# vsu/foo-dsp-bfir

Hardware: AMD Instinct MI355X
Metric: Msamples/s (output channel-samples), 8ch 131072-tap FIR @4096-sample partitions (higher is better)
Workload: dtype f32; 1 GPU; cfg3_8ch_131072tap_L4096_fp32; channels=8, taps=131072, partition=4096, fft_size=8192, partitions=32, blocks_per_launch=4096, engines_rank0=1, channels_rank0=8, streams_total=1, io=interleaved frames resident in HBM (generated there), parallelism=one independent stream per rank, no collective

## Files before the change

### foo-dsp-bfir_amd/csrc/engine.hip

```cpp
#include <hip/hip_runtime.h>

#include <algorithm>
#include <climits>
#include <cmath>
#include <cstdarg>
#include <cstdio>
#include <cstdlib>
#include <cstring>
#include <cstdint>
#include <thread>
#include <type_traits>
#include <vector>

#include "../../include/bfir_hip.h"
#include "kernels.h"

using namespace bfir;

static bfir_log_fn g_log = nullptr;

extern "C" void bfir_set_log_callback(bfir_log_fn fn) { g_log = fn; }

void bfir_logf(const char *fmt, ...)
{
// ... 54 lines not shown
    int Co = 0, GCo = 0;
    bool mimo = false, mimo_mac = false;
    int in_bytes = 0, out_bytes = 0, in_fmt = 0, out_fmt = 0;
    double in_scale = 1.0, out_scale = 1.0, of_max = 1.0;
    FftPlan plan;
    bool big = false;
    BigPlan bplan;
    int chunk = 0, ring = 0;
    int want_chunk = 0;
    void *H = nullptr, *X = nullptr, *Y = nullptr, *tout = nullptr;
    void *tin[2] = {nullptr, nullptr};
    void *Yb[2] = {nullptr, nullptr};
    void *saved[2] = {nullptr, nullptr};
    BlockRef hist[2];
    int *d_nblk = nullptr;
    DevOverflow *d_of = nullptr;
    int *d_bad = nullptr;
    std::vector<int> nblk;
    std::vector<char> eng_init;
    unsigned long long blockcounter = 0;
    unsigned long long chunk_seq = 0;
    int curbuf = 0;
    hipStream_t stream = nullptr, s_front = nullptr, s_mac = nullptr, s_in = nullptr, s_out = nullptr;
    hipEvent_t ev_entry = nullptr, ev_fwd[2] = {nullptr, nullptr}, ev_mac[2] = {nullptr, nullptr};
    hipEvent_t ev_inv[2] = {nullptr, nullptr};
    bool pipe3 = true;
    bool ilv = false;
    bool pair = false;
    bool pair_tp = false;
    bool pair_cap = false;
    bool direct = false;
    FftPlan plan2;
    void *H2 = nullptr;
    int *d_nblk2 = nullptr;
    std::vector<int> nblk2;
    int fade_len = 0, fade_pos = 0;
    float fade_f = 0.f; double fade_d = 0.0;
    bool fade_fused = false;
    bool pair_new = false;
    bool fade_patch = false;
    int *d_patch = nullptr; size_t patch_ints = 0;
    bool patch_fused = false;
    void *bank = nullptr;
    std::vector<int> bank_nb;
    int *d_gather = nullptr; size_t gather_ints = 0;
    void *Yf[2] = {nullptr, nullptr};
    int yf_blocks = 0;
    void *ft[2] = {nullptr, nullptr};
    int ft_blocks = 0;
    float *tails[2][2] = {{nullptr, nullptr}, {nullptr, nullptr}};
    const float *hist_raw[2] = {nullptr, nullptr};
    int8_t *d_dither_tab = nullptr; int dither_size = 0;
    DevDitherState *d_dither_state = nullptr;
    bool inline_launch = false;
    bool async_pending = false;
    int *h_bad = nullptr;
    int *bad_host_cur = nullptr;
    bool serial = false;
    void *pin_in[2] = {nullptr, nullptr}, *pin_out[2] = {nullptr, nullptr};
    void *dev_in[2] = {nullptr, nullptr}, *dev_out[2] = {nullptr, nullptr};
    hipEvent_t ev_h2d[2] = {nullptr, nullptr}, ev_comp[2] = {nullptr, nullptr}, ev_d2h[2] = {nullptr, nullptr};
    size_t stage_bytes_in = 0, stage_bytes_out = 0;
    bool nup = false, nup_tail = false;
    bool levels = false;
    bool mlevels = false;
    bool back_fused = false;
    int n_tail = 0;
    bfir_engine *tail[BFIR_MAX_LEVELS - 1] = {nullptr, nullptr, nullptr};
    int lv_r[BFIR_MAX_LEVELS - 1] = {0, 0, 0}, lv_D[BFIR_MAX_LEVELS - 1] = {0, 0, 0};
    bool lv_active[BFIR_MAX_LEVELS - 1] = {false, false, false};
    int nup_mask = 0;
    void *pbuf = nullptr;
    long long pbuf_upto = 0;
    hipEvent_t ev_nup = nullptr;
    void *zring = nullptr; int zblocks = 0;
    long long z_from = 0, z_next = 0;
    int ring_extra = 0;
    void *zring2 = nullptr;
    int lf_mode = 0; long long lf_j1 = -1;
    bool lf_stop = false;
    bool mfade_duo = true;
    int inv_quad = -1;
    int fwd_wide = -1;
    bool profiling = false;
    struct Span { int k; hipEvent_t a, b; };
    std::vector<Span> spans;
    std::vector<hipEvent_t> ev_pool;
    double prof_ms[BFIR_K_COUNT] = {0, 0, 0, 0, 0};
    long prof_n[BFIR_K_COUNT] = {0, 0, 0, 0, 0};
    struct DelaySide {
        bool on = false;
        int max_delay = 0, steps = 0, h = 0;
        double beta = 0.0;
        long H = 0;
        void *hist[2] = {nullptr, nullptr}; int cur = 0;
        void *scratch = nullptr; size_t scratch_bytes = 0;
        void *d_tab = nullptr;
        std::vector<int> delay, sub;
    };
    DelaySide dly[2];
    hipEvent_t ev_dly = nullptr;
    hipEvent_t ev_dly_done = nullptr; hipStream_t dly_stream = nullptr;
};

static size_t cbuf_bytes(const bfir_engine *e) { return (size_t)e->N * (size_t)e->s; }

static bfir_engine *level(const bfir_engine *e, int k) { return k == 0 ? const_cast<bfir_engine *>(e) : e->tail[k - 1]; }

static void delay_free(bfir_engine *e, int side)
{
    bfir_engine::DelaySide &d = e->dly[side];
    void *bufs[] = {d.hist[0], d.hist[1], d.scratch, d.d_tab};
    for (void *b : bufs) if (b) (void)hipFree(b);
    d = bfir_engine::DelaySide();
}

static int materialise_history(bfir_engine *e)
{
    HIP_TRY(hipDeviceSynchronize());
    const size_t Ls = (size_t)e->L * e->s;
    for (int i = 0; i < 2; i++) {
        if (e->hist[i].ptr != e->saved[i])
            HIP_TRY(hipMemcpy2D(e->saved[i], Ls, e->hist[i].ptr, (size_t)e->hist[i].ch_stride * e->s, Ls, e->GC,
                                hipMemcpyDeviceToDevice));
        e->hist[i].ptr = e->saved[i];
        e->hist[i].ch_stride = e->L;
    }
    HIP_TRY(hipDeviceSynchronize());
    return BFIR_OK;
}

static void free_staging(bfir_engine *e)
{
    for (int i = 0; i < 2; i++) {
        if (e->pin_in[i]) (void)hipHostFree(e->pin_in[i]);
        if (e->pin_out[i]) (void)hipHostFree(e->pin_out[i]);
        if (e->dev_in[i]) (void)hipFree(e->dev_in[i]);
        if (e->dev_out[i]) (void)hipFree(e->dev_out[i]);
        e->pin_in[i] = e->pin_out[i] = e->dev_in[i] = e->dev_out[i] = nullptr;
    }
    e->stage_bytes_in = e->stage_bytes_out = 0;
}

static void free_work(bfir_engine *e)
{
    void **bufs[] = {&e->X, &e->Yb[0], &e->Yb[1], &e->tin[0], &e->tin[1], &e->tout};
    for (void **b : bufs) { if (*b) (void)hipFree(*b); *b = nullptr; }
    free_staging(e);
    e->chunk = e->ring = 0;
    if (e->h_bad) { (void)hipHostFree(e->h_bad); e->h_bad = nullptr; }
}

static int alloc_work(bfir_engine *e, int chunk)
{
    const size_t cb = cbuf_bytes(e);
    const int ring = 2 * chunk + e->B + e->ring_extra;
    if (e->X) { int rc = materialise_history(e); if (rc != BFIR_OK) return rc; }
    void *X = nullptr, *Y0 = nullptr, *Y1 = nullptr, *tin0 = nullptr, *tin1 = nullptr, *tout = nullptr;
    HIP_TRY(hipMalloc(&X, (size_t)e->GC * ring * cb));
    HIP_TRY(hipMalloc(&Y0, (size_t)e->GCo * chunk * cb));
    HIP_TRY(hipMalloc(&Y1, (size_t)e->GCo * chunk * cb));
    if (e->nup && !e->back_fused) HIP_TRY(hipMalloc(&tout, (size_t)e->GCo * chunk * e->L * e->s));
    if (!e->pair && !e->direct) {
        HIP_TRY(hipMalloc(&tin0, (size_t)e->GC * chunk * e->L * e->s));
        HIP_TRY(hipMalloc(&tin1, (size_t)e->GC * chunk * e->L * e->s));
        HIP_TRY(hipMalloc(&tout, (size_t)e->GCo * chunk * e->L * e->s));
    }
    HIP_TRY(hipMemset(X, 0, (size_t)e->GC * ring * cb));
    if (e->X) {
        const int keep = (int)std::min<unsigned long long>(e->blockcounter, (unsigned long long)(e->B - 1 + e->ring_extra));
        for (int d = 1; d <= keep; d++) {
            const unsigned long long j = e->blockcounter - d;
            const size_t so = (size_t)(j % e->ring) * cb, dn = (size_t)(j % ring) * cb;
            HIP_TRY(hipMemcpy2D((char *)X + dn, (size_t)ring * cb, (char *)e->X + so, (size_t)e->ring * cb, cb,
                                e->GC, hipMemcpyDeviceToDevice));
        }
    }
    HIP_TRY(hipDeviceSynchronize());
    free_work(e);
    e->X = X; e->Yb[0] = Y0; e->Yb[1] = Y1; e->tin[0] = tin0; e->tin[1] = tin1; e->tout = tout;
    e->chunk = chunk; e->ring = ring;
    return BFIR_OK;
}

static void choose_path(bfir_engine *e)
{
    e->ilv = e->s == 4 && e->N >= 512;
    const char *pv = getenv("BFIR_PAIR");
    const char *tv = getenv("BFIR_PAIR_TIME");
    const bool tp_ok = !(tv && atoi(tv) == 0);
    e->pair_tp = (e->C % 2) == 1 && tp_ok;
    e->pair = e->ilv && e->in_fmt == 8 && e->out_fmt == 8 && ((e->C % 2) == 0 || e->pair_tp) &&
              pair_supported(e->L) && !(pv && atoi(pv) == 0);
    e->pair_tp = e->pair_tp && e->pair;
    if (e->matrix) {
        const bool split = e->nup || e->nup_tail;
        e->pair = e->pair && e->C % 2 == 0 && (split || e->Co % 2 == 0);
        e->pair_tp = false;
        e->pair_cap = e->pair;
    }
    const char *dv = getenv("BFIR_DIRECT");
    const bool stereo = e->in_bytes == 4 && e->out_bytes == 4 && (e->C % 2) == 0 && !e->ilv &&
                        direct_stereo_supported(e->L, e->s);
    const bool wide = (e->in_bytes == 8 && e->out_bytes == 8) || e->C == 1 || stereo || run64_supported(e->L, e->s);
    e->direct = !e->pair && fmt_is_native(e->in_fmt) && fmt_is_native(e->out_fmt) && !(pv && atoi(pv) == 0) &&
                (dv ? atoi(dv) != 0 : wide);
    if (e->matrix) e->direct = !e->pair;
    if (e->big) e->pair = e->pair_tp = e->direct = false;
    if (e->nup || e->nup_tail) {
        e->pair = e->pair && !e->pair_tp;
        e->pair_tp = false;
        e->direct = !e->pair;
        e->back_fused = e->nup && (e->matrix ? e->s == 4 && e->ilv && e->out_fmt == BFIR_SAMPLE_FORMAT_FLOAT_LE && pair_supported(e->L)
                                             : e->pair);
    }
    {
        const char *fp = getenv("BFIR_F64_PAIRS"), *ms = getenv("BFIR_MAC_SYS");
        const bool other_mac = (ms && atoi(ms) == 0) || getenv("BFIR_MAC_BATCHED");
        if (e->s == 8 && e->direct && pairs64_supported(e->L, e->s) && e->B <= BFIR_MAC_SYS_MAX_B && !other_mac &&
            !(fp && atoi(fp) == 0))
            e->ilv = true;
    }
    if (const char *mv = getenv("BFIR_MFADE_DUO")) e->mfade_duo = atoi(mv) != 0;
    if (const char *pf = getenv("BFIR_PATCH_FUSED")) e->patch_fused = atoi(pf) != 0;
    if (e->mimo) {
        const char *mm = getenv("BFIR_MIMO_MAC");
        e->mimo_mac = e->C > BFIR_MAT_MAX || e->Co > BFIR_MAT_MAX || (mm && atoi(mm) != 0);
    }
    if (const char *qv = getenv("BFIR_INV_QUAD")) e->inv_quad = atoi(qv) != 0;
    if (const char *wv = getenv("BFIR_FWD_WIDE")) e->fwd_wide = atoi(wv) != 0;
    if (const char *pm = getenv("BFIR_PIPE")) { e->pipe3 = atoi(pm) >= 3; e->serial = atoi(pm) == 1; }
    else if (e->s == 8) { e->pipe3 = false; e->serial = true; }
}

static void log_creation(const bfir_engine *e)
{
    char shape[64];
    if (e->big) {
        bfir_logf("bfir engine: big, %d x %d channels, partition %d = %d x %d, %d blocks, realsize %d on device %d. layout=%s",
                  e->n_eng, e->C, e->L, 1 << e->bplan.log2m1, 1 << e->bplan.log2m2, e->B, e->s, e->device, e->ilv ? "pairs" : "grouped");
        return;
    }
    if (e->matrix) snprintf(shape, sizeof(shape), "%s %d -> %d", e->mimo ? "mimo" : "matrix", e->C, e->Co);
    else snprintf(shape, sizeof(shape), "%d x %d channels", e->n_eng, e->C);
    bfir_logf("bfir engine: %s, partition %d, %d blocks, realsize %d on device %d. path=%s layout=%s run=%s",
              shape, e->L, e->B, e->s, e->device,
              e->pair_tp ? "time-pair" : e->pair ? "pair" : e->direct ? "direct" : "staging", e->ilv ? "pairs" : "grouped",
              e->s == 8 && e->direct && run64_supported(e->L, e->s) ? "on" : "off");
}

static bfir_engine *engine_create(int n_engines, int filter_length, int filter_blocks, int realsize, int channels,
                                  int channels_out, bool matrix, int in_format, int out_format, int sampling_rate,
                                  int apply_dither, int device, int *err, int nup_level = 0, int ring_extra = 0, bool big = false,
                                  int max_channels = BFIR_MAXCHANNELS)
{
    const bool mimo = matrix && max_channels > BFIR_MAXCHANNELS;
    int dummy;
    if (!err) err = &dummy;
    *err = BFIR_OK;
    if (channels < 1 || channels > max_channels || channels_out < 1 || channels_out > max_channels) {
        bfir_logf("Number of channels (%d) exceeds limit (%d).", std::max(channels, channels_out), max_channels);
        *err = BFIR_ERR_ARG; return nullptr;
    }
    if (realsize != 4 && realsize != 8) { bfir_logf("Invalid real size %d.", realsize); *err = BFIR_ERR_ARG; return nullptr; }
    if (filter_length < 1 || (filter_length & (filter_length - 1))) {
        bfir_logf("Invalid length %d.", filter_length); *err = BFIR_ERR_ARG; return nullptr;
    }
    if (filter_blocks < 1 || n_engines < 1) { *err = BFIR_ERR_ARG; return nullptr; }
    if (!fmt_bytes(in_format) || !fmt_bytes(out_format)) { *err = BFIR_ERR_UNSUPPORTED; return nullptr; }
    int ndev = bfir_device_count();
    if (ndev <= 0) { *err = BFIR_ERR_NO_DEVICE; return nullptr; }
    if (device < 0 || device >= ndev) { *err = BFIR_ERR_ARG; return nullptr; }
    if (hipSetDevice(device) != hipSuccess) { *err = BFIR_ERR_HIP; return nullptr; }

    bfir_engine *e = new bfir_engine();
    e->device = device;
    e->L = filter_length; e->N = 2 * filter_length; e->B = filter_blocks; e->s = realsize;
    e->C = channels; e->n_eng = n_engines; e->GC = n_engines * channels;
    e->matrix = matrix; e->Co = channels_out; e->GCo = n_engines * channels_out;
    e->mimo = mimo;
    e->in_bytes = fmt_bytes(in_format); e->out_bytes = fmt_bytes(out_format);
    e->in_fmt = in_format; e->out_fmt = out_format;
    e->in_scale = fmt_info(in_format).isfloat ? 1.0 : 1.0 / fmt_full_scale(in_format);
    e->out_scale = fmt_info(out_format).isfloat ? 1.0 : fmt_full_scale(out_format);
    e->of_max = fmt_info(out_format).isfloat ? 1.0 : fmt_full_scale(out_format) - 1.0;
    e->nup = nup_level == 1; e->nup_tail = nup_level == 2;
    e->ring_extra = ring_extra;
    e->big = big;
    choose_path(e);
    e->nblk.assign(matrix ? (size_t)e->Co * e->C : (size_t)e->GC, 0);
    e->eng_init.assign(n_engines, 0);
    int rc = big ? big_plan_create(&e->bplan, filter_length, realsize) : fft_plan_create(&e->plan, filter_length, realsize);
    if (rc != 0) { *err = (rc == -1) ? BFIR_ERR_UNSUPPORTED : BFIR_ERR_HIP; delete e; return nullptr; }
    auto fail = [&](int code) { *err = code; bfir_engine_destroy(e); return (bfir_engine *)nullptr; };
    if (e->pair || e->direct) {
        if ((e->pair || e->back_fused) && fft_plan_create(&e->plan2, 2 * filter_length, 4) != 0) return fail(BFIR_ERR_HIP);
        const size_t tb = (size_t)e->n_eng * e->L * e->C * e->in_bytes;
        for (int st = 0; st < 2; st++)
            for (int i = 0; i < 2; i++) {
                if (hipMalloc((void **)&e->tails[st][i], tb) != hipSuccess) return fail(BFIR_ERR_HIP);
                (void)hipMemset(e->tails[st][i], 0, tb);
            }
        e->hist_raw[0] = e->tails[1][0]; e->hist_raw[1] = e->tails[1][1];
    }
    hipStream_t *streams[] = {&e->stream, &e->s_front, &e->s_mac, &e->s_in, &e->s_out};
    for (hipStream_t *st : streams)
        if (hipStreamCreateWithFlags(st, hipStreamNonBlocking) != hipSuccess) return fail(BFIR_ERR_HIP);
    hipEvent_t *events[] = {&e->ev_entry, &e->ev_fwd[0], &e->ev_fwd[1], &e->ev_mac[0], &e->ev_mac[1],
                            &e->ev_inv[0], &e->ev_inv[1],
                            &e->ev_h2d[0], &e->ev_h2d[1], &e->ev_comp[0], &e->ev_comp[1], &e->ev_d2h[0], &e->ev_d2h[1]};
    for (hipEvent_t *ev : events)
        if (hipEventCreateWithFlags(ev, hipEventDisableTiming) != hipSuccess) return fail(BFIR_ERR_HIP);
    const size_t cb = cbuf_bytes(e), Ls = (size_t)e->L * e->s;
// ... 1370 lines not shown
    d.h2 = e->H2;
    d.row = e->d_patch; d.ent = e->d_patch + e->Co + 1;
    d.y2 = Y2; d.y2_ch_stride = y2_ch_stride;
    return d;
}

static int patch_chunk_ok(const bfir_engine *e, int tc)
{
    const long ys = (long)e->chunk * e->N;
    if (!patch_supported(patch_args(e, 0, nullptr, nullptr, 0, tc)) ||
        (chunk_takes_wpatch(e) && !wpatch_supported(wpatch_args(e, 0, nullptr, ys, nullptr, 0, tc)))) {
        bfir_logf("bfir engine: %d fading blocks per launch are past the pair-list kernel's grid.", tc);
        return BFIR_ERR_UNSUPPORTED;
    }
    return BFIR_OK;
}

static int queue_mac_patch(bfir_engine *e, int base_slot, void *Y, long y_ch_stride, void *Y2, long y2_ch_stride, int tc,
                           hipStream_t s, bool spans)
{
    const bool prof = e->profiling;
    if (!spans) e->profiling = false;
    int rc;
    if (chunk_takes_wpatch(e)) {
        ProfScope ps(e, BFIR_K_MAC, s);
        rc = launch_wpatch(wpatch_args(e, base_slot, Y, y_ch_stride, Y2, y2_ch_stride, tc), s) != 0 ? BFIR_ERR_UNSUPPORTED : BFIR_OK;
    } else {
        {
            ProfScope ps(e, BFIR_K_MAC, s);
            rc = queue_mac(e, base_slot, Y, y_ch_stride, tc, false, s);
        }
        if (rc == BFIR_OK) {
            ProfScope ps(e, BFIR_K_MAC, s);
            PatchArgs a = patch_args(e, base_slot, Y, Y2, y2_ch_stride, tc);
            a.y_ch_stride = y_ch_stride;
            rc = launch_patch(a, s) != 0 ? BFIR_ERR_UNSUPPORTED : BFIR_OK;
        }
    }
    e->profiling = prof;
    return rc;
}

static int chunk_aligned(const bfir_engine *e, Path p, const Chunk &c)
{
    const uintptr_t out_mask = (e->pair_tp || (e->matrix && (e->Co & 1))) ? 3 : 7;
    if (p == Path::Pair &&
        ((((uintptr_t)c.d_in | (uintptr_t)c.in_stride) & (e->pair_tp ? 3 : 7)) || (((uintptr_t)c.d_out | (uintptr_t)c.out_stride) & out_mask))) {
        bfir_logf("bfir engine: frame buffers of the float fast path must be 8-byte aligned (4 with an odd channel count).");
        return BFIR_ERR_ARG;
    }
    if (p == Path::Direct && (((uintptr_t)c.d_in | (uintptr_t)c.in_stride) % e->in_bytes ||
                              ((uintptr_t)c.d_out | (uintptr_t)c.out_stride) % e->out_bytes)) {
        bfir_logf("bfir engine: frame buffers must be aligned to their sample size.");
        return BFIR_ERR_ARG;
    }
    return BFIR_OK;
}

static void queue_stage_in(bfir_engine *e, const Chunk &c, hipStream_t sf)
{
    ProfScope ps(e, BFIR_K_STAGE_IN, sf);
    StageInArgs a;
    a.raw = c.d_in; a.eng_stride_bytes = c.in_stride; a.frame_off = c.frame_off;
    a.n_eng = e->n_eng; a.C = e->C; a.raw_bytes = e->in_bytes; a.spacing = e->C; a.fmt = e->in_fmt;
    a.n_frames = (long)c.tc * e->L;
    a.dst = e->tin[c.par]; a.dst_ch_stride = (long)e->chunk * e->L; a.dst_off = 0;
    a.realsize = e->s;
    launch_stage_in(a, sf);
}

static void queue_fwd(bfir_engine *e, Path p, const Chunk &c, hipStream_t sf)
{
    ProfScope ps(e, BFIR_K_FWD, sf);
    if (p == Path::Pair) {
        FwdPairArgs a;
        a.raw = (const float *)c.d_in; a.eng_stride = c.in_stride / 4; a.frame_off = c.frame_off;
        a.C = e->C; a.n_eng = e->n_eng; a.n_t = c.tc;
        a.prev = e->hist_raw[e->curbuf];
        a.save_last = e->tails[c.par][c.idx_last]; a.save_prev = e->tails[c.par][1 ^ c.idx_last];
        a.carry = e->hist_raw[1 ^ c.idx_last];
        a.hist_eng_stride = (long)e->L * e->C;
        a.dst = (float *)e->X; a.dst_ch_stride = (long)e->ring * e->N; a.ring = e->ring; a.base_slot = c.base_slot;
        a.scale = (float)e->in_scale;
        a.tp = e->pair_tp; a.wide = e->fwd_wide;
        launch_fwd_pair(e->plan2, a, sf);
    } else {
        FwdArgs a;
        a.dst = e->X; a.dst_ch_stride = (long)e->ring * e->N; a.ring = e->ring; a.base_slot = c.base_slot;
        a.n_t = c.tc; a.n_ch = e->GC;
        a.load_scale = 1.0; a.out_scale = e->in_scale; a.zero_first_half = 0; a.interleaved = e->ilv;
        if (p == Path::Direct) {
            a.src = nullptr; a.src_ch_stride = 0; a.prev = nullptr; a.prev_ch_stride = 0;
            a.raw_bytes = e->in_bytes; a.raw = c.d_in; a.raw_eng_stride = c.in_stride / e->in_bytes; a.frame_off = c.frame_off; a.C = e->C;
            a.prev_raw = e->hist_raw[e->curbuf];
            a.save_last = e->tails[c.par][c.idx_last]; a.save_prev = e->tails[c.par][1 ^ c.idx_last];
            a.carry = e->hist_raw[1 ^ c.idx_last];
            a.hist_eng_stride = (long)e->L * e->C;
        } else {
            a.src = e->tin[c.par]; a.src_ch_stride = (long)e->chunk * e->L;
            a.prev = e->hist[e->curbuf].ptr; a.prev_ch_stride = e->hist[e->curbuf].ch_stride;
        }
        queue_transform_fwd(e, a, sf);
    }
    if (p != Path::Staging) { e->hist_raw[0] = e->tails[c.par][0]; e->hist_raw[1] = e->tails[c.par][1]; }
}

static InvStats inv_stats(const bfir_engine *e, const Chunk &c)
{
    return InvStats{(float)e->of_max, e->d_of, e->GCo, e->d_bad, c.block_base, e->bad_host_cur};
}

static int chunk_rings(const bfir_engine *e, LevelRing (&ring)[BFIR_LEVEL_RINGS], const void **z_new = nullptr)
{
    int nr = 0;
    for (int i = 0; i < e->n_tail; i++) {
        if (!(e->nup_mask >> i & 1)) continue;
        const bfir_engine *t = e->tail[i];
        if (z_new) z_new[nr] = t->lf_mode ? t->zring2 : t->zring;
        LevelRing &g = ring[nr++];
        g.z = t->zring; g.zlen = g.z_ch_stride = (long)t->zblocks * t->L;
        g.m0 = ((long long)e->blockcounter - e->lv_D[i]) * e->L; g.m_min = t->z_from * (long long)t->L;
        g.m0r = (long)(((g.m0 % g.zlen) + g.zlen) % g.zlen);
    }
    if (!nr) ring[0] = LevelRing{nullptr, 0, 0, 0, 0, 0};
    for (int k = std::max(nr, 1); k < BFIR_LEVEL_RINGS; k++) { ring[k] = ring[0]; if (z_new) z_new[k] = z_new[0]; }
    return nr;
}

static void queue_inv_lone(bfir_engine *e, const Chunk &c, const LevelRing (&ring)[BFIR_LEVEL_RINGS], int nr, hipStream_t st)
{
    LoneInvArgs a;
    a.ch = e->Co & ~1;
    a.y = (const float *)c.Y + (long)a.ch * e->chunk * e->N;
    for (int k = 0; k < BFIR_LEVEL_RINGS; k++) a.ring[k] = ring[k];
    a.n_rings = nr;
    a.raw = (float *)c.d_out; a.frame_off = c.frame_off;
    a.frame_stride = e->Co; a.n_t = c.tc;
    a.scale = (float)e->out_scale; a.st = inv_stats(e, c);
    launch_inv_lone(e->plan2, a, st);
}

static void queue_inv(bfir_engine *e, Path p, const Chunk &c, hipStream_t st)
{
    ProfScope ps(e, BFIR_K_INV, st);
    if (p == Path::Pair) {
        InvPairArgs a;
        a.y = (const float *)c.Y; a.y_ch_stride = (long)e->chunk * e->N;
        a.raw = (float *)c.d_out; a.eng_stride = c.out_stride / 4; a.frame_off = c.frame_off;
        a.C = e->Co; a.n_eng = e->n_eng; a.n_t = c.tc;
        a.scale = (float)e->out_scale; a.max = (float)e->of_max;
        a.overflow = e->d_of; a.of_shard_stride = e->GCo; a.bad_block = e->d_bad; a.block_base = c.block_base; a.bad_host = e->bad_host_cur;
        a.tp = e->pair_tp; a.quad = e->inv_quad;
        if (e->matrix && (e->Co & 1)) {
            a.C = e->Co & ~1; a.frame_stride = e->Co;
            LevelRing none[BFIR_LEVEL_RINGS] = {};
            queue_inv_lone(e, c, none, 0, st);
        }
        launch_inv_pair(e->plan2, a, st);
        return;
    }
    InvArgs a;
    a.src = c.Y; a.src_ch_stride = (long)e->chunk * e->N;
    a.n_t = c.tc;
    a.in_scale = e->out_scale; a.full_output = 0; a.interleaved = e->ilv;
    if (p == Path::Direct) {
        a.dst = nullptr; a.dst_ch_stride = 0; a.n_ch = e->GCo;
        a.raw_bytes = e->out_bytes; a.raw = c.d_out; a.raw_eng_stride = c.out_stride / e->out_bytes; a.frame_off = c.frame_off; a.C = e->Co;
// ... 1133 lines not shown
```

### foo-dsp-bfir_amd/csrc/kernels.h

```cpp
#pragma once
#include <hip/hip_runtime.h>
#include <stdint.h>
#include <stdlib.h>

#include <vector>

namespace bfir {

struct DevOverflow {
    unsigned int n_overflows;
    int intlargest;
    unsigned long long largest_bits;
};
constexpr int BFIR_OF_SHARDS = 64;
__device__ __forceinline__ DevOverflow *of_shard(DevOverflow *base, long shard_stride)
{
    return base + (long)(blockIdx.x & (BFIR_OF_SHARDS - 1)) * shard_stride;
}

__device__ __forceinline__ int xcd_work_item(int b, int W)
{
    const int xcd = b & 7, qn = W >> 3, rn = W & 7;
    return (xcd < rn ? xcd * (qn + 1) : rn * (qn + 1) + (xcd - rn) * qn) + (b >> 3);
}
// ... 146 lines not shown
    void *y2; long y2_ch_stride;
    int n_t, n_in, n_out, N, realsize;
    int interleaved;
};
bool patch_supported(const PatchArgs &a);
int launch_patch(const PatchArgs &a, hipStream_t s);

struct WpatchArgs {
    MimoArgs a;
    const void *h2;
    const int *row, *ent;
    void *y2; long y2_ch_stride;
};
inline __host__ __device__ PatchArgs wpatch_patch_args(const WpatchArgs &d)
{
    PatchArgs p;
    p.x = d.a.x; p.x_ch_stride = d.a.x_ch_stride; p.ring = d.a.ring; p.base_slot = d.a.base_slot;
    p.h = d.a.h; p.h2 = d.h2; p.h_pair_stride = d.a.h_pair_stride;
    p.row = d.row; p.ent = d.ent;
    p.y = d.a.y; p.y_ch_stride = d.a.y_ch_stride;
    p.y2 = d.y2; p.y2_ch_stride = d.y2_ch_stride;
    p.n_t = d.a.n_t; p.n_in = d.a.n_in; p.n_out = d.a.n_out; p.N = d.a.N; p.realsize = d.a.realsize;
    p.interleaved = d.a.interleaved;
    return p;
}
bool wpatch_supported(const WpatchArgs &d);
int launch_wpatch(const WpatchArgs &d, hipStream_t s);

struct BankArgs {
    const void *bank; void *dst;
    const int *tab;
    int n_rows;
    unsigned long long row_bytes, part_bytes;
};
constexpr int BFIR_BANK_SPAN = 4096;
constexpr int BFIR_BANK_STEPS = 4;
bool bank_gather_supported(const BankArgs &a);
int launch_bank_gather(const BankArgs &a, hipStream_t s);

struct InvArgs {
    const void *src; long src_ch_stride;
    void *dst; long dst_ch_stride;
    int n_t, n_ch;
    double in_scale;
    int full_output;
    int interleaved = 0;
    int raw_bytes = 0;
    void *raw = nullptr; long raw_eng_stride = 0, frame_off = 0; int C = 0;
    double max = 1.0; DevOverflow *overflow = nullptr; int *bad_block = nullptr; int block_base = 0;
    int *bad_host = nullptr;
    long of_shard_stride = 0;
};
void launch_inv(const FftPlan &plan, const InvArgs &a, hipStream_t s);

struct BigPlan {
    int log2m = 0, log2m1 = 0, log2m2 = 0;
    int realsize = 0;
    FftPlan p1, p2;
    void *t_hi = nullptr, *t_lo = nullptr;
    void *s_hi = nullptr, *s_lo = nullptr;
};
bool big_split(int filter_length, int realsize, int *log2m1, int *log2m2);
int  big_plan_create(BigPlan *plan, int filter_length, int realsize);
void big_plan_destroy(BigPlan *plan);
bool big_launch_fits(const BigPlan &plan, int n_t, int n_ch);
void launch_fwd_big(const BigPlan &plan, const FwdArgs &a, hipStream_t s);
void launch_inv_big(const BigPlan &plan, const InvArgs &a, hipStream_t s);

bool pair_supported(int filter_length);
bool direct_stereo_supported(int filter_length, int realsize);
bool run64_supported(int filter_length, int realsize);
bool pairs64_supported(int filter_length, int realsize);
struct FwdPairArgs {
    const float *raw; long eng_stride; long frame_off;
    int C, n_eng, n_t;
    const float *prev;
    float *save_last, *save_prev;
    const float *carry;
    long hist_eng_stride;
    float *dst; long dst_ch_stride; int ring, base_slot;
    float scale;
    int tp = 0;
    int wide = -1;
};
void launch_fwd_pair(const FftPlan &plan, const FwdPairArgs &a, hipStream_t s);
bool launch_fwd_wide(const FftPlan &plan, const FwdPairArgs &a, hipStream_t s);
struct InvPairArgs {
    const float *y; long y_ch_stride;
    float *raw; long eng_stride; long frame_off;
    int C, n_eng, n_t;
    float scale, max;
    DevOverflow *overflow; int *bad_block; int block_base;
    int *bad_host = nullptr;
    long of_shard_stride = 0;
    int tp = 0;
    int frame_stride = 0;
    int quad = -1;
};
void launch_inv_pair(const FftPlan &plan, const InvPairArgs &a, hipStream_t s);
bool launch_inv_quad(const FftPlan &plan, const InvPairArgs &a, hipStream_t s);

struct InvStats {
    float max;
    DevOverflow *overflow; long of_shard_stride;
    int *bad_block; int block_base; int *bad_host;
};
#define BFIR_PLANAR_KERNELS(k) k<float, 4>, k<float, 1>, k<double, 2>, k<double, 1>
template <typename A>
inline void launch_planar(void (*f4)(A), void (*f1)(A), void (*d2)(A), void (*d1)(A), const A &a, bool aligned, hipStream_t s)
{
    const long lanes = aligned ? a.n / (16 / a.realsize) : a.n;
    const dim3 grid((unsigned)((lanes + 255) / 256), (unsigned)a.n_ch), block(256);
    hipLaunchKernelGGL(a.realsize == 4 ? (aligned ? f4 : f1) : (aligned ? d2 : d1), grid, block, 0, s, a);
}

struct FadeInvArgs {
    const float *y_old; long y_old_ch_stride;
    const float *y_new; long y_new_ch_stride;
    float *raw; long frame_off;
    int n_ch, n_t;
    float scale;
    float f; int m0;
    InvStats st;
};
void launch_inv_fade(const FftPlan &plan, const FadeInvArgs &a, hipStream_t s);
struct FadeBlendArgs {
    void *y_old; const void *y_new; long ch_stride;
    int n_ch; long n;
    double f; int m0;
    int realsize;
};
void launch_fade_blend(const FadeBlendArgs &a, hipStream_t s);

constexpr int BFIR_LEVEL_RINGS = 3;
struct LevelRing {
    const void *z; long z_ch_stride; long zlen;
    long long m0, m_min; long m0r;
};
struct LevelsInvArgs {
    const float *y; long y_ch_stride;
    LevelRing ring[BFIR_LEVEL_RINGS]; int n_rings;
    float *raw; long frame_off;
    int n_ch, n_t;
    float scale;
    InvStats st;
    int frame_stride = 0;
};
void launch_inv_nup(const FftPlan &plan, const LevelsInvArgs &a, hipStream_t s);
void launch_inv_levels(const FftPlan &plan, const LevelsInvArgs &a, hipStream_t s);
struct LevelsCombineArgs {
    void *y; long y_ch_stride;
    LevelRing ring[BFIR_LEVEL_RINGS]; int n_rings;
    int n_ch; long n;
    int realsize;
};
void launch_nup_combine(const LevelsCombineArgs &a, hipStream_t s);
void launch_levels_combine(const LevelsCombineArgs &a, hipStream_t s);
inline bool rings_aligned16(const LevelRing *ring, const void *const *z_new, int n_rings, int vec)
{
    bool ok = true;
    for (int r = 0; r < n_rings; r++)
        ok = ok && ring[r].z_ch_stride % vec == 0 && ring[r].zlen % vec == 0 && ring[r].m0r % vec == 0 &&
             ((uintptr_t)ring[r].z | (uintptr_t)(z_new ? z_new[r] : nullptr)) % 16 == 0;
    return ok;
}

// ... 67 lines not shown
```

### foo-dsp-bfir_amd/csrc/wide.hip

```cpp
#include "kernels.h"

#include <algorithm>
#include <atomic>
#include <cstdint>
#include <cstdlib>

#include "fft_lds.h"
#include "pair_io.h"

namespace bfir {

namespace {

constexpr int WIDE_PF_PASS = 1;

__device__ __forceinline__ void asm_prefetch8x4_out(u32x4 (&d)[8], unsigned voff, i32x4 r, unsigned step)
{
    const unsigned s1 = __builtin_amdgcn_readfirstlane(step), s2 = 2 * s1, s3 = 3 * s1, s4 = 4 * s1, s5 = 5 * s1, s6 = 6 * s1, s7 = 7 * s1;
    asm volatile("s_nop 4\n\t"
                 "buffer_load_dwordx4 %0, %8, %9, 0 offen\n\t"
                 "buffer_load_dwordx4 %1, %8, %9, %10 offen\n\t"
                 "buffer_load_dwordx4 %2, %8, %9, %11 offen\n\t"
                 "buffer_load_dwordx4 %3, %8, %9, %12 offen\n\t"
                 "buffer_load_dwordx4 %4, %8, %9, %13 offen\n\t"
                 "buffer_load_dwordx4 %5, %8, %9, %14 offen\n\t"
                 "buffer_load_dwordx4 %6, %8, %9, %15 offen\n\t"
                 "buffer_load_dwordx4 %7, %8, %9, %16 offen"
                 : "=&v"(d[0]), "=&v"(d[1]), "=&v"(d[2]), "=&v"(d[3]), "=&v"(d[4]), "=&v"(d[5]), "=&v"(d[6]), "=&v"(d[7])
                 : "v"(voff), "s"(r), "s"(s1), "s"(s2), "s"(s3), "s"(s4), "s"(s5), "s"(s6), "s"(s7)
                 : "memory");
}

template <int LOG2N>
__global__ __launch_bounds__(FftCfg<LOG2N>::NT, 4) void k_fwd_wide_ps(FwdPairArgs a, const float2 *__restrict__ twb, int run_len)
{
    using F = LdsFft<float, LOG2N, -1>;
    constexpr int N = F::M, NT = F::NT, P = F::P, L = N / 2, H = P / 2;
    static_assert(F::radix(0) == 16 && P == 16, "in_index(tid, e) = tid + e * (N / 16)");
    static_assert(F::phys(32) == 33 && F::phys(N - 1) == N - 1 + N / 32 - 1, "the split step's addresses assume i + (i >> 5)");
    static_assert(WIDE_PF_PASS >= 1 && WIDE_PF_PASS < F::NP, "the prefetch goes under one of the passes behind the first");
    __shared__ __attribute__((aligned(16))) float2 lds[F::LDS_ELEMS + 1];
    __shared__ __attribute__((aligned(16))) float2 ldsb[F::LDSB_ELEMS];

    const int tid = threadIdx.x;
    const int w = xcd_work_item(blockIdx.x, gridDim.x);
    const int quarter_c = a.C / 4, units = a.n_eng * quarter_c;
    const int rr = w / units, pp = w - rr * units;
    const float sc = 0.5f * a.scale;
    const int g = pp / quarter_c, cq = pp - g * quarter_c;
    const int C = a.C;
    const int t0 = rr * run_len, t1 = min(a.n_t, t0 + run_len);
    if (t0 >= t1) return;

    float2 B[F::NBREG];
    F::load_bases(B, ldsb, twb, tid);

    const float *__restrict__ raw = a.raw + (long)g * a.eng_stride + a.frame_off * C + 4 * cq;
    const long hist = (long)g * a.hist_eng_stride + 4 * cq;
    const unsigned blk_bytes = (unsigned)L * C * 4u;
    const unsigned fo = (unsigned)tid * (unsigned)C * 4u;
    const unsigned estep = (unsigned)NT * C * 4u;
    static_assert(H == 8, "the prefetch statement moves eight 16-byte pieces per thread");
    float4 cur[H];
    u32x4 nxt[H];
    {
        const __amdgpu_buffer_rsrc_t ro = make_rsrc((t0 == 0) ? a.prev + hist : raw + (long)(t0 - 1) * L * C, blk_bytes);
#pragma unroll
        for (int e = 0; e < H; e++) {
            const float4 v = buf_load4(ro, fo, e * estep);
            cur[e].x = v.x * sc; cur[e].y = v.y * sc; cur[e].z = v.z * sc; cur[e].w = v.w * sc;
        }
        if (a.n_t == 1) {
            const __amdgpu_buffer_rsrc_t rc = make_rsrc(a.carry + hist, blk_bytes);
            u32x4 mv[H];
#pragma unroll
            for (int e = 0; e < H; e++) mv[e] = __builtin_amdgcn_raw_buffer_load_b128(rc, fo, e * estep, 0);
            asm_store8x4(mv, fo, make_rsrc_words(a.save_prev + hist, blk_bytes), estep);
        }
        const __amdgpu_buffer_rsrc_t rb = make_rsrc(raw + (long)t0 * L * C, blk_bytes);
#pragma unroll
        for (int e = 0; e < H; e++) nxt[e] = __builtin_amdgcn_raw_buffer_load_b128(rb, fo, e * estep, 0);
#pragma unroll
        for (int e = 0; e < H; e++) asm volatile("" : "+v"(nxt[e]));
    }
    float *__restrict__ da0 = a.dst + (long)(g * C + 4 * cq) * a.dst_ch_stride;
    for (int t = t0; t < t1; t++) {
        asm_wait_vmcnt<2 * (P / 4)>(nxt);
        if (t >= a.n_t - 2) {
            asm_store8x4(nxt, fo, make_rsrc_words((t == a.n_t - 1 ? a.save_last : a.save_prev) + hist, blk_bytes), estep);
        }
        unsigned bx[H], by[H];
#pragma unroll
        for (int e = 0; e < H; e++) { bx[e] = nxt[e].z; by[e] = nxt[e].w; }
        static_for<0, 2>([&](auto PR_) {
            constexpr int PR = decltype(PR_)::value;
            float re[P], im[P];
#pragma unroll
            for (int e = 0; e < H; e++) {
                if constexpr (PR == 0) {
                    re[e] = cur[e].x; im[e] = cur[e].y;
                    cur[e].x = __uint_as_float(nxt[e].x) * sc; cur[e].y = __uint_as_float(nxt[e].y) * sc;
                    re[H + e] = cur[e].x; im[H + e] = cur[e].y;
                } else {
                    re[e] = cur[e].z; im[e] = cur[e].w;
                    cur[e].z = __uint_as_float(bx[e]) * sc; cur[e].w = __uint_as_float(by[e]) * sc;
                    re[H + e] = cur[e].z; im[H + e] = cur[e].w;
                }
            }
            {
                float2 w0[1];
                F::template butterflies<0>(re, im, w0);
            }
            static_for<1, F::NP>([&](auto S_) {
                constexpr int S = decltype(S_)::value;
                int tl = tid; asm volatile("" : "+v"(tl));
                F::template exchange<S - 1>(re, im, lds, tl);
                F::template butterflies_tb<S>(re, im, B, ldsb, tl);
                if constexpr (PR == 1 && S == WIDE_PF_PASS) {
                    asm_prefetch8x4_out(nxt, fo, make_rsrc_words(raw + (long)(t + 1) * L * C, t + 1 < t1 ? blk_bytes : 0u), estep);
                }
            });

            int tz = tid; asm volatile("" : "+v"(tz));
            __syncthreads();
            {
                float2 *zw = lds + F::phys(tz);
                static_for<0, P>([&](auto E_) {
                    constexpr int e = decltype(E_)::value;
                    static_assert(F::out_index(0, e) % 32 == 0, "additive padding");
                    float2 v; v.x = re[e]; v.y = im[e];
                    zw[F::phys(F::out_index(0, e))] = v;
                });
            }
            __syncthreads();
            const long slot = (long)((a.base_slot + t) % a.ring) * N;
            float *da = da0 + (long)(2 * PR) * a.dst_ch_stride + slot;
            const __amdgpu_buffer_rsrc_t rxa = make_rsrc(da, (unsigned)N * 4u), rxb = make_rsrc(da + a.dst_ch_stride, (unsigned)N * 4u);
            const float2 *zk = lds + F::phys(2 * tz);
            constexpr int OMAX = F::phys(2 * NT * (P / 4 - 1));
            const float2 *zn1 = lds + (F::phys(N - 1 - 2 * tz) - OMAX);
            const float2 *zn0 = zn1 + ((tz & 15) == 0 ? 2 : 1);
#pragma unroll
            for (int j = 0; j < P / 4; j++) {
                if (j > 0) __builtin_amdgcn_sched_barrier(0);
                const int o = F::phys(2 * NT * j);
                const float2 zk0 = zk[o], zk1 = zk[o + 1];
                const float2 zn0v = zn0[OMAX - o], zn1v = zn1[OMAX - o];
                float4 xa, xb;
                xa.x = zk0.x + zn0v.x; xa.y = zk0.y - zn0v.y;
                xb.x = zk0.y + zn0v.y; xb.y = zn0v.x - zk0.x;
                xa.z = zk1.x + zn1v.x; xa.w = zk1.y - zn1v.y;
                xb.z = zk1.y + zn1v.y; xb.w = zn1v.x - zk1.x;
                if (j == 0) {
                    const float2 zh = lds[F::phys(L)];
                    const bool k0 = tz == 0;
                    xa.x = k0 ? 2.f * zk0.x : xa.x; xa.y = k0 ? 2.f * zh.x : xa.y;
                    xb.x = k0 ? 2.f * zk0.y : xb.x; xb.y = k0 ? 2.f * zh.y : xb.y;
                }
                buf_store4<2>(rxa, (unsigned)tz * 16u, (unsigned)(j * NT) * 16u, xa);
                buf_store4<2>(rxb, (unsigned)tz * 16u, (unsigned)(j * NT) * 16u, xb);
            }
        });
    }
    asm_wait_vmcnt<0>(nxt);
}

}

#define BFIR_FOR_WIDE_LOG2N(F) F(13) F(14)

static std::atomic<int64_t> g_wide_launches{0};

static int wide_run_len(int n_t, int units)
{
    if (const char *e = getenv("BFIR_WIDE_RUN_FWD")) return std::max(1, atoi(e));
    const int slots = 512;
    const int runs = std::max(1, slots / std::max(1, units));
    const int fill = std::max(1, (n_t + runs - 1) / runs);
    return std::min(fill, 4);
}

static bool wide_pays(int log2m) { return log2m == 13; }

bool launch_fwd_wide(const FftPlan &plan, const FwdPairArgs &a, hipStream_t s)
{
    if (a.tp || a.wide == 0 || a.C <= 0 || a.C % 4 != 0) return false;
    const uintptr_t ptrs = (uintptr_t)a.raw | (uintptr_t)a.prev | (uintptr_t)a.save_last | (uintptr_t)a.save_prev | (uintptr_t)a.carry;
    if ((ptrs & 15u) != 0 || (a.eng_stride & 3) != 0 || (a.hist_eng_stride & 3) != 0) return false;
    const int units = a.n_eng * (a.C / 4);
    if (a.n_t <= 0 || units <= 0 || !plan.twb) return false;
    if (a.wide < 0 && ((long)a.n_t * units < 512 || !wide_pays(plan.log2m))) return false;
    const int len = wide_run_len(a.n_t, units), runs = (a.n_t + len - 1) / len;
    switch (plan.log2m) {
#define F(lg) case lg: hipLaunchKernelGGL((k_fwd_wide_ps<lg>), dim3(runs * units), dim3(FftCfg<lg>::NT), 0, s, a, (const float2 *)plan.twb, len); break;
        BFIR_FOR_WIDE_LOG2N(F)
#undef F
        default: return false;
    }
    g_wide_launches.fetch_add(1, std::memory_order_relaxed);
    return true;
}

}

extern "C" int64_t bfir_fwd_wide_launches(void) { return bfir::g_wide_launches.load(std::memory_order_relaxed); }
```

Baseline: 122,100 Msamples/s.

## Alternate forward-FFT run direction per block so adjacent runs share boundary blocks

Splits the wide forward-FFT kernel body into a templated run routine that can walk its time blocks forward or backward. A new zigzag kernel gives odd runs the descending direction, so neighbouring runs touch their shared boundary input blocks at about the same time, and the history-save stores are placed for the reverse walk. The default run length is cut from 4 to 3 when zigzag is on, which raises the block count for more parallelism. The descending path adds complexity in the tail-history handling and shifts the load-versus-compute balance per block.

```diff
diff --git a/foo-dsp-bfir_amd/csrc/engine.hip b/foo-dsp-bfir_amd/csrc/engine.hip
--- a/foo-dsp-bfir_amd/csrc/engine.hip
+++ b/foo-dsp-bfir_amd/csrc/engine.hip
@@ -160,6 +160,7 @@
     bool mfade_duo = true;
     int inv_quad = -1;
     int fwd_wide = -1;
+    int fwd_zigzag = 1;
     bool profiling = false;
     struct Span { int k; hipEvent_t a, b; };
     std::vector<Span> spans;
@@ -307,6 +308,7 @@
     }
     if (const char *qv = getenv("BFIR_INV_QUAD")) e->inv_quad = atoi(qv) != 0;
     if (const char *wv = getenv("BFIR_FWD_WIDE")) e->fwd_wide = atoi(wv) != 0;
+    if (const char *zv = getenv("BFIR_FWD_ZIGZAG")) e->fwd_zigzag = atoi(zv) != 0;
     if (const char *pm = getenv("BFIR_PIPE")) { e->pipe3 = atoi(pm) >= 3; e->serial = atoi(pm) == 1; }
     else if (e->s == 8) { e->pipe3 = false; e->serial = true; }
 }
@@ -1843,7 +1845,7 @@
         a.hist_eng_stride = (long)e->L * e->C;
         a.dst = (float *)e->X; a.dst_ch_stride = (long)e->ring * e->N; a.ring = e->ring; a.base_slot = c.base_slot;
         a.scale = (float)e->in_scale;
-        a.tp = e->pair_tp; a.wide = e->fwd_wide;
+        a.tp = e->pair_tp; a.wide = e->fwd_wide; a.zigzag = e->fwd_zigzag;
         launch_fwd_pair(e->plan2, a, sf);
     } else {
         FwdArgs a;
diff --git a/foo-dsp-bfir_amd/csrc/kernels.h b/foo-dsp-bfir_amd/csrc/kernels.h
--- a/foo-dsp-bfir_amd/csrc/kernels.h
+++ b/foo-dsp-bfir_amd/csrc/kernels.h
@@ -252,6 +252,7 @@
     float scale;
     int tp = 0;
     int wide = -1;
+    int zigzag = 1;
 };
 void launch_fwd_pair(const FftPlan &plan, const FwdPairArgs &a, hipStream_t s);
 bool launch_fwd_wide(const FftPlan &plan, const FwdPairArgs &a, hipStream_t s);
diff --git a/foo-dsp-bfir_amd/csrc/wide.hip b/foo-dsp-bfir_amd/csrc/wide.hip
--- a/foo-dsp-bfir_amd/csrc/wide.hip
+++ b/foo-dsp-bfir_amd/csrc/wide.hip
@@ -31,26 +31,19 @@
                  : "memory");
 }
 
-template <int LOG2N>
-__global__ __launch_bounds__(FftCfg<LOG2N>::NT, 4) void k_fwd_wide_ps(FwdPairArgs a, const float2 *__restrict__ twb, int run_len)
+template <int LOG2N, bool DESC>
+__device__ __forceinline__ void wide_run(const FwdPairArgs &a, const float2 *__restrict__ twb, float2 *lds, float2 *ldsb,
+                                         const int t0, const int t1, const int g, const int cq)
 {
     using F = LdsFft<float, LOG2N, -1>;
     constexpr int N = F::M, NT = F::NT, P = F::P, L = N / 2, H = P / 2;
     static_assert(F::radix(0) == 16 && P == 16, "in_index(tid, e) = tid + e * (N / 16)");
     static_assert(F::phys(32) == 33 && F::phys(N - 1) == N - 1 + N / 32 - 1, "the split step's addresses assume i + (i >> 5)");
     static_assert(WIDE_PF_PASS >= 1 && WIDE_PF_PASS < F::NP, "the prefetch goes under one of the passes behind the first");
-    __shared__ __attribute__((aligned(16))) float2 lds[F::LDS_ELEMS + 1];
-    __shared__ __attribute__((aligned(16))) float2 ldsb[F::LDSB_ELEMS];
 
     const int tid = threadIdx.x;
-    const int w = xcd_work_item(blockIdx.x, gridDim.x);
-    const int quarter_c = a.C / 4, units = a.n_eng * quarter_c;
-    const int rr = w / units, pp = w - rr * units;
     const float sc = 0.5f * a.scale;
-    const int g = pp / quarter_c, cq = pp - g * quarter_c;
     const int C = a.C;
-    const int t0 = rr * run_len, t1 = min(a.n_t, t0 + run_len);
-    if (t0 >= t1) return;
 
     float2 B[F::NBREG];
     F::load_bases(B, ldsb, twb, tid);
@@ -63,7 +56,24 @@
     static_assert(H == 8, "the prefetch statement moves eight 16-byte pieces per thread");
     float4 cur[H];
     u32x4 nxt[H];
-    {
+    if constexpr (DESC) {
+        const __amdgpu_buffer_rsrc_t rt = make_rsrc(raw + (long)(t1 - 1) * L * C, blk_bytes);
+        u32x4 top[H];
+#pragma unroll
+        for (int e = 0; e < H; e++) top[e] = __builtin_amdgcn_raw_buffer_load_b128(rt, fo, e * estep, 0);
+        if (t1 - 1 >= a.n_t - 2)
+            asm_store8x4(top, fo, make_rsrc_words((t1 - 1 == a.n_t - 1 ? a.save_last : a.save_prev) + hist, blk_bytes), estep);
+        const __amdgpu_buffer_rsrc_t rb = make_rsrc(raw + (long)(t1 - 2) * L * C, blk_bytes);
+#pragma unroll
+        for (int e = 0; e < H; e++) nxt[e] = __builtin_amdgcn_raw_buffer_load_b128(rb, fo, e * estep, 0);
+#pragma unroll
+        for (int e = 0; e < H; e++) {
+            cur[e].x = __uint_as_float(top[e].x) * sc; cur[e].y = __uint_as_float(top[e].y) * sc;
+            cur[e].z = __uint_as_float(top[e].z) * sc; cur[e].w = __uint_as_float(top[e].w) * sc;
+        }
+#pragma unroll
+        for (int e = 0; e < H; e++) asm volatile("" : "+v"(nxt[e]));
+    } else {
         const __amdgpu_buffer_rsrc_t ro = make_rsrc((t0 == 0) ? a.prev + hist : raw + (long)(t0 - 1) * L * C, blk_bytes);
 #pragma unroll
         for (int e = 0; e < H; e++) {
@@ -84,9 +94,11 @@
         for (int e = 0; e < H; e++) asm volatile("" : "+v"(nxt[e]));
     }
     float *__restrict__ da0 = a.dst + (long)(g * C + 4 * cq) * a.dst_ch_stride;
-    for (int t = t0; t < t1; t++) {
+    for (int t = DESC ? t1 - 1 : t0; DESC ? t >= t0 : t < t1; t += DESC ? -1 : 1) {
         asm_wait_vmcnt<2 * (P / 4)>(nxt);
-        if (t >= a.n_t - 2) {
+        if constexpr (DESC) {
+            if (t - 1 == a.n_t - 2 && t > t0) asm_store8x4(nxt, fo, make_rsrc_words(a.save_prev + hist, blk_bytes), estep);
+        } else if (t >= a.n_t - 2) {
             asm_store8x4(nxt, fo, make_rsrc_words((t == a.n_t - 1 ? a.save_last : a.save_prev) + hist, blk_bytes), estep);
         }
         unsigned bx[H], by[H];
@@ -94,17 +106,18 @@
         for (int e = 0; e < H; e++) { bx[e] = nxt[e].z; by[e] = nxt[e].w; }
         static_for<0, 2>([&](auto PR_) {
             constexpr int PR = decltype(PR_)::value;
+            constexpr int KEPT = DESC ? H : 0, NEW = DESC ? 0 : H;
             float re[P], im[P];
 #pragma unroll
             for (int e = 0; e < H; e++) {
                 if constexpr (PR == 0) {
-                    re[e] = cur[e].x; im[e] = cur[e].y;
+                    re[KEPT + e] = cur[e].x; im[KEPT + e] = cur[e].y;
                     cur[e].x = __uint_as_float(nxt[e].x) * sc; cur[e].y = __uint_as_float(nxt[e].y) * sc;
-                    re[H + e] = cur[e].x; im[H + e] = cur[e].y;
+                    re[NEW + e] = cur[e].x; im[NEW + e] = cur[e].y;
                 } else {
-                    re[e] = cur[e].z; im[e] = cur[e].w;
+                    re[KEPT + e] = cur[e].z; im[KEPT + e] = cur[e].w;
                     cur[e].z = __uint_as_float(bx[e]) * sc; cur[e].w = __uint_as_float(by[e]) * sc;
-                    re[H + e] = cur[e].z; im[H + e] = cur[e].w;
+                    re[NEW + e] = cur[e].z; im[NEW + e] = cur[e].w;
                 }
             }
             {
@@ -117,7 +130,10 @@
                 F::template exchange<S - 1>(re, im, lds, tl);
                 F::template butterflies_tb<S>(re, im, B, ldsb, tl);
                 if constexpr (PR == 1 && S == WIDE_PF_PASS) {
-                    asm_prefetch8x4_out(nxt, fo, make_rsrc_words(raw + (long)(t + 1) * L * C, t + 1 < t1 ? blk_bytes : 0u), estep);
+                    if constexpr (DESC)
+                        asm_prefetch8x4_out(nxt, fo, make_rsrc_words(raw + (long)(t - 2) * L * C, t > t0 ? blk_bytes : 0u), estep);
+                    else
+                        asm_prefetch8x4_out(nxt, fo, make_rsrc_words(raw + (long)(t + 1) * L * C, t + 1 < t1 ? blk_bytes : 0u), estep);
                 }
             });
 
@@ -165,19 +181,56 @@
     asm_wait_vmcnt<0>(nxt);
 }
 
+struct WideItem { int run, g, cq, t0, t1; };
+__device__ __forceinline__ WideItem wide_work_item(const FwdPairArgs &a, int run_len)
+{
+    const int w = xcd_work_item(blockIdx.x, gridDim.x);
+    const int quarter_c = a.C / 4, units = a.n_eng * quarter_c;
+    WideItem i;
+    i.run = w / units;
+    const int pp = w - i.run * units;
+    i.g = pp / quarter_c; i.cq = pp - i.g * quarter_c;
+    i.t0 = i.run * run_len; i.t1 = min(a.n_t, i.t0 + run_len);
+    return i;
+}
+
+template <int LOG2N>
+__global__ __launch_bounds__(FftCfg<LOG2N>::NT, 4) void k_fwd_wide_ps(FwdPairArgs a, const float2 *__restrict__ twb, int run_len)
+{
+    using F = LdsFft<float, LOG2N, -1>;
+    __shared__ __attribute__((aligned(16))) float2 lds[F::LDS_ELEMS + 1];
+    __shared__ __attribute__((aligned(16))) float2 ldsb[F::LDSB_ELEMS];
+    const WideItem i = wide_work_item(a, run_len);
+    if (i.t0 >= i.t1) return;
+    wide_run<LOG2N, false>(a, twb, lds, ldsb, i.t0, i.t1, i.g, i.cq);
+}
+
+template <int LOG2N>
+__global__ __launch_bounds__(FftCfg<LOG2N>::NT, 4) void k_fwd_zig_ps(FwdPairArgs a, const float2 *__restrict__ twb, int run_len)
+{
+    using F = LdsFft<float, LOG2N, -1>;
+    __shared__ __attribute__((aligned(16))) float2 lds[F::LDS_ELEMS + 1];
+    __shared__ __attribute__((aligned(16))) float2 ldsb[F::LDSB_ELEMS];
+    const WideItem i = wide_work_item(a, run_len);
+    if (i.t0 >= i.t1) return;
+    if (i.run & 1) wide_run<LOG2N, true>(a, twb, lds, ldsb, i.t0, i.t1, i.g, i.cq);
+    else wide_run<LOG2N, false>(a, twb, lds, ldsb, i.t0, i.t1, i.g, i.cq);
+}
+
 }
 
 #define BFIR_FOR_WIDE_LOG2N(F) F(13) F(14)
 
 static std::atomic<int64_t> g_wide_launches{0};
-
-static int wide_run_len(int n_t, int units)
+static std::atomic<int64_t> g_zigzag_launches{0};
+
+static int wide_run_len(int n_t, int units, bool zigzag)
 {
     if (const char *e = getenv("BFIR_WIDE_RUN_FWD")) return std::max(1, atoi(e));
     const int slots = 512;
     const int runs = std::max(1, slots / std::max(1, units));
     const int fill = std::max(1, (n_t + runs - 1) / runs);
-    return std::min(fill, 4);
+    return std::min(fill, zigzag ? 3 : 4);
 }
 
 static bool wide_pays(int log2m) { return log2m == 13; }
@@ -190,17 +243,23 @@
     const int units = a.n_eng * (a.C / 4);
     if (a.n_t <= 0 || units <= 0 || !plan.twb) return false;
     if (a.wide < 0 && ((long)a.n_t * units < 512 || !wide_pays(plan.log2m))) return false;
-    const int len = wide_run_len(a.n_t, units), runs = (a.n_t + len - 1) / len;
+    const int len = wide_run_len(a.n_t, units, a.zigzag != 0), runs = (a.n_t + len - 1) / len;
+    const bool zig = a.zigzag != 0 && runs > 1;
     switch (plan.log2m) {
-#define F(lg) case lg: hipLaunchKernelGGL((k_fwd_wide_ps<lg>), dim3(runs * units), dim3(FftCfg<lg>::NT), 0, s, a, (const float2 *)plan.twb, len); break;
+#define F(lg) case lg:                                                                                                            \
+        if (zig) hipLaunchKernelGGL((k_fwd_zig_ps<lg>), dim3(runs * units), dim3(FftCfg<lg>::NT), 0, s, a, (const float2 *)plan.twb, len); \
+        else hipLaunchKernelGGL((k_fwd_wide_ps<lg>), dim3(runs * units), dim3(FftCfg<lg>::NT), 0, s, a, (const float2 *)plan.twb, len);    \
+        break;
         BFIR_FOR_WIDE_LOG2N(F)
 #undef F
         default: return false;
     }
     g_wide_launches.fetch_add(1, std::memory_order_relaxed);
+    if (zig) g_zigzag_launches.fetch_add(1, std::memory_order_relaxed);
     return true;
 }
 
 }
 
 extern "C" int64_t bfir_fwd_wide_launches(void) { return bfir::g_wide_launches.load(std::memory_order_relaxed); }
+extern "C" int64_t bfir_fwd_zigzag_launches(void) { return bfir::g_zigzag_launches.load(std::memory_order_relaxed); }
```

Result: no change. 121,600 Msamples/s (-0.4%).
